# liortalker/MindTheEdge

Measured on AMD Instinct MI355X. Metric: training images/sec, PackNet-SAN+edge-loss 384x1280 bf16, higher is better.
Workload: dtype bf16; 1 GPU; T8: PackNet-SAN + silog + 4-scale depth-edge loss training step, 384x1280, 8 frames/GPU, dropout 0.5, flip 0.5; global_batch=8, height=384, width=1280, parallelism=single GPU

## Files before the change

### include/mte_kernels.h

```cpp
#ifndef MTE_KERNELS_H
#define MTE_KERNELS_H

#ifdef __cplusplus
extern "C" {
#endif

typedef struct ihipStream_t* mte_stream_t;

#define MTE_OK 0
#define MTE_ERR_ARG (-1)
#define MTE_ERR_LAUNCH (-2)
#define MTE_ERR_UNSUPPORTED (-3)
#define MTE_DT_BF16 0
#define MTE_DT_F32 1

#define MTE_CONV_ACCUMULATE 1
#define MTE_CONV_SOLO 2
int mte_conv2d_igemm(const void* x, long ldx, const void* wpack, const float* bias, void* y, long ldy, int out_f32,
                     int B, int H, int W, int Cin_p, int N, int KH, int KW, int dtype,
                     float* workspace, long workspace_elems, int accumulate, mte_stream_t stream);
int mte_conv2d_igemm_unshuffle(const void* x, long ldx, const void* wpack, void* y, long ldy,
                               int B, int H, int W, int Cin_p, int N, int KH, int KW, int dtype, int accumulate, mte_stream_t stream);
#define MTE_OPT_GN_PREZEROED 0
#define MTE_OPT_LOSS_PREZEROED 1
#define MTE_OPT_HANDOFF_FENCES 2
#define MTE_OPT_WGRAD_SHARES_CHIP 3
int mte_set_option(int option, int value);
#define MTE_DEVERR_GN_CLUSTER_FWD 1
#define MTE_DEVERR_GN_CLUSTER_BWD 2
#define MTE_DEVERR_IMAGE_RESAMPLE 4
int mte_device_error_init(void);
int mte_device_error_poll(void);
int mte_conv2d_wgrad(const void* x, long ldx, const void* dy, long ldy, float* dw_stage, int stage_parts, int* parts_out,
                     int B, int H, int W, int Cin_p, int N, int KH, int KW, int dtype, mte_stream_t stream);
int mte_conv2d_wgrad_nine_tap(int H, int W, int Cin_p, int N, int KH, int KW, int dtype);
int mte_pack_conv_weights(const float* w_oihw, void* wfwd, void* wbwd, int Cout, int Cin, int KH, int KW,
                          int Cin_p, int Cout_p, int dtype, mte_stream_t stream);
typedef struct { const float* w; void* wf; void* wb; void* pf; void* pb; int Cout, Cin, taps, Cin_p; int end_f, end_b, end_pf, end_pb; } mte_pack_job;
int mte_pack_conv_weights_multi(const void* jobs, int njobs, int dtype, mte_stream_t stream);
int mte_pack_conv_weights_bwd(const void* wfwd, void* wbwd, int Cout, int KH, int KW, int Cin_p, int dtype, mte_stream_t stream);
int mte_unpack_conv_wgrad(float* dw_stage, int parts, float* dw_oihw, int Cout, int Cin, int KH, int KW, int Cin_p, mte_stream_t stream);
int mte_colsum(const void* y, long ld, long M, int N, float* out, int dtype, mte_stream_t stream);

int mte_conv2d_patch_supported(int W, int Cin_p, int N, int KH, int KW, int dtype);
int mte_conv2d_patch_wgrad_supported(int W, int Cin_p, int N, int KH, int KW, int dtype);
long mte_conv2d_patch_pack_elems(int Cin_p, int N, int KH, int KW);
int mte_conv2d_patch_repack(const void* wgeneric, void* wpatch, int Cin_p, int N, int KH, int KW, mte_stream_t stream);
int mte_conv2d_patch_fwd(const void* x, long ldx, const void* wpatch, const float* bias, void* y, long ldy,
                         int B, int H, int W, int Cin_p, int N, int KH, int KW, int accumulate, mte_stream_t stream);
int mte_conv2d_patch_wgrad(const void* x, long ldx, const void* dy, long lddy, float* dw_stage, int stage_parts, int* parts_out,
                           int B, int H, int W, int Cin_p, int N, int KH, int KW, mte_stream_t stream);
long mte_conv2d_patch_fwd_gn_elems(int B, int H, int W);
int mte_conv2d_patch_fwd_gn(const void* x, long ldx, const void* wpatch, const float* bias, void* y, long ldy, int B, int H, int W, int Cin_p, int N, int KH, int KW,
                            int accumulate, float* rec, long rec_elems, int* tiles_per_sample_out, mte_stream_t stream);

int mte_conv2d_stem_supported(int W, int Cin_p, int N, int KH, int KW, int dtype);
int mte_conv2d_stem_fwd(const void* x, long ldx, const void* wf, const float* bias, void* y, long ldy,
                        int B, int H, int W, int N, int KH, int KW, mte_stream_t stream);
int mte_conv2d_stem_wgrad(const void* x, long ldx, const void* dy, long lddy, float* dw_stage, int stage_parts, int* parts_out,
                          int B, int H, int W, int N, int KH, int KW, mte_stream_t stream);

long mte_gn_stats_elems(int B);
// ... 279 lines not shown
```

### mindtheedge_amd/csrc/conv_igemm.hip

```cpp
#include "common.hpp"
#include "conv_args.hpp"

#ifdef MTE_STAMPS
__device__ unsigned long long g_igemm_stamps[16384 * 8];
extern "C" int mtei_igemm_stamps(unsigned long long* host, int n) {
    return hipMemcpyFromSymbol(host, HIP_SYMBOL(g_igemm_stamps), sizeof(unsigned long long) * n) == hipSuccess ? 0 : -1;
}
#endif

namespace {


template <typename T> struct Mma;
template <> struct Mma<bf16_t> {
    __device__ static __forceinline__ void run(const u32x4_t& a, const u32x4_t& b, f32x16_t& c) {
        c = __builtin_amdgcn_mfma_f32_32x32x16_bf16(__builtin_bit_cast(bf16x8_t, a), __builtin_bit_cast(bf16x8_t, b), c, 0, 0, 0);
    }
};
template <> struct Mma<float> {
    __device__ static __forceinline__ void run(const u32x4_t& a, const u32x4_t& b, f32x16_t& c) {
#pragma unroll
        for (int i = 0; i < 4; ++i)
            c = __builtin_amdgcn_mfma_f32_32x32x2f32(__uint_as_float(a[i]), __uint_as_float(b[i]), c, 0, 0, 0);
    }
// ... 1141 lines not shown

template <typename T>
__global__ __launch_bounds__(256) void pack_weights_bwd_kernel(const T* __restrict__ wf, T* __restrict__ wb,
                                                               int Cout, int taps, int Cin_p, int Cout_p) {
    __shared__ T tile[64][64 + 2];
    const int Kp = taps * Cin_p;
    const int n0 = blockIdx.x * 64, k0 = blockIdx.y * 64;
    for (int i = threadIdx.x; i < 64 * 64; i += 256) {
        const int r = i >> 6, cidx = i & 63;
        const int n = n0 + r, k = k0 + cidx;
        tile[r][cidx] = (n < Cout && k < Kp) ? wf[(long)n * Kp + k] : (T)0;
    }
    __syncthreads();
    for (int i = threadIdx.x; i < 64 * 64; i += 256) {
        const int kk = i >> 6, nn = i & 63;
        const int k = k0 + kk, n = n0 + nn;
        if (k < Kp && n < Cout_p) {
            const int tap = k / Cin_p, c = k - tap * Cin_p;
            wb[((long)c * taps + (taps - 1 - tap)) * Cout_p + n] = n < Cout ? tile[nn][kk] : (T)0;
        }
    }
}

struct PackJob {
    const float* w;
    void* wf;
    void* wb;
    void* pf;
    void* pb;
    int Cout, Cin, taps, Cin_p;
    int end_f, end_b, end_pf, end_pb;
};
constexpr int PACK_JOBS_MAX = 48;
struct PackTable { int n; int pad_; PackJob j[PACK_JOBS_MAX]; };
constexpr int PACK_FRAG_PER_BLOCK = 256 * 8;

template <typename T> __device__ __forceinline__ void store8(T* dst, const float* v);
template <> __device__ __forceinline__ void store8<bf16_t>(bf16_t* dst, const float* v) { *(u32x4_t*)dst = pack16<bf16_t>(v); }
template <> __device__ __forceinline__ void store8<float>(float* dst, const float* v) {
    *(u32x4_t*)dst = pack16<float>(v); *(u32x4_t*)(dst + 4) = pack16<float>(v + 4);
}

__host__ __device__ inline int pack_fn(int taps) { const int f = (64 * 65) / (64 * taps); return f < 1 ? 1 : (f > 16 ? 16 : f); }

template <typename T>
__global__ __launch_bounds__(256) void pack_multi_kernel(const PackTable tb) {
    __shared__ float s_w[64 * 65];
    int ji = 0;
    while (ji + 1 < tb.n && (int)blockIdx.x >= tb.j[ji].end_pb) ++ji;
    const PackJob& J = tb.j[ji];
    const int start = ji ? tb.j[ji - 1].end_pb : 0;
    const int bid = blockIdx.x;
    const int Cout = J.Cout, Cin = J.Cin, taps = J.taps, Cin_p = J.Cin_p;
    const float* __restrict__ w = J.w;
    if (bid < J.end_f) {
        const int fn = pack_fn(taps);
        const int cchunks = (Cin_p + 63) >> 6;
        const int lb = bid - start, n0 = (lb / cchunks) * fn, c0 = (lb - (lb / cchunks) * cchunks) * 64;
        const int nc = min(64, Cin - c0), nn = min(fn, Cout - n0);
        const int run = nc > 0 ? nc * taps : 0, rs = 64 * taps;
        for (int i = threadIdx.x; i < nn * run; i += 256) {
            const int ni = i / run, r = i - ni * run;
            s_w[ni * rs + r] = w[((long)(n0 + ni) * Cin + c0) * taps + r];
        }
        __syncthreads();
        const int ncp = min(64, Cin_p - c0), nch = ncp >> 3;
        T* wf = (T*)J.wf;
        for (int i = threadIdx.x; i < nn * taps * nch; i += 256) {
            const int ch8 = i % nch, t2 = i / nch, tap = t2 % taps, ni = t2 / taps;
            float v[8];
#pragma unroll
            for (int j = 0; j < 8; ++j) {
                const int cl = ch8 * 8 + j;
                v[j] = cl < nc ? s_w[ni * rs + cl * taps + tap] : 0.f;
            }
            store8<T>(wf + ((long)(n0 + ni) * taps + tap) * Cin_p + c0 + ch8 * 8, v);
        }
        return;
    }
    if (bid < J.end_b) {
        const int Kp = taps * Cin_p, Kr = taps * Cin;
        const int ktiles = (Kp + 63) >> 6;
        const int lb = bid - J.end_f, n0 = (lb / ktiles) * 64, k0 = (lb % ktiles) * 64;
        for (int i = threadIdx.x; i < 64 * 64; i += 256) {
            const int r = i >> 6, kk = i & 63;
            const int n = n0 + r, k = k0 + kk;
            s_w[r * 65 + kk] = (n < Cout && k < Kr) ? w[(long)n * Kr + k] : 0.f;
        }
        __syncthreads();
        T* wb = (T*)J.wb;
        if (Cout % 8 == 0) {
            for (int i = threadIdx.x; i < 64 * 8; i += 256) {
                const int kk = i >> 3, n8 = i & 7;
                const int k = k0 + kk, n = n0 + n8 * 8;
                if (k < Kp && n < Cout) {
                    const int c = k / taps, tap = k - c * taps;
                    float v[8];
#pragma unroll
                    for (int j = 0; j < 8; ++j) v[j] = s_w[(n8 * 8 + j) * 65 + kk];
                    store8<T>(wb + ((long)c * taps + (taps - 1 - tap)) * Cout + n, v);
                }
            }
            return;
        }
        for (int i = threadIdx.x; i < 64 * 64; i += 256) {
            const int kk = i >> 6, nn = i & 63;
            const int k = k0 + kk, n = n0 + nn;
            if (k < Kp && n < Cout) {
                const int c = k / taps, tap = k - c * taps;
                Elem<T>::st(wb + ((long)c * taps + (taps - 1 - tap)) * Cout + n, s_w[nn * 65 + kk]);
            }
        }
        return;
    }
    const bool fwd = bid < J.end_pf;
    const int N = fwd ? Cout : Cin_p, C = fwd ? Cin_p : Cout;
    const int NT = (N + 31) >> 5;
    const long total8 = (long)((C + 31) >> 5) * taps * 2 * NT * 64;
    const long i8 = (long)(bid - (fwd ? J.end_b : J.end_pf)) * 256 + threadIdx.x;
    if (i8 >= total8) return;
    long t = i8;
    const int lane = (int)(t & 63); t >>= 6;
    const int nt = (int)(t % NT); t /= NT;
    const int kk = (int)(t & 1); t >>= 1;
    const int tap = (int)(t % taps); const int sl = (int)(t / taps);
    const int n = nt * 32 + (lane & 31), c0 = sl * 32 + kk * 16 + (lane >> 5) * 8;
    float v[8];
#pragma unroll
    for (int j = 0; j < 8; ++j) {
        const int c = c0 + j;
        float x = 0.f;
        if (n < N && c < C) {
            if (fwd) { if (c < Cin) x = w[((long)n * Cin + c) * taps + tap]; }
            else if (n < Cin) x = w[((long)c * Cin + n) * taps + (taps - 1 - tap)];
        }
        v[j] = x;
    }
    store8<T>((T*)(fwd ? J.pf : J.pb) + i8 * 8, v);
}

__global__ __launch_bounds__(256) void unpack_wgrad_kernel(const float* __restrict__ st, float* __restrict__ dw, int Cout, int Cin, int taps, int Cin_p, int parts) {
    extern __shared__ float s_t[];
    const int n = blockIdx.x, c0 = blockIdx.y * 64;
    const int nc = min(64, Cin - c0);
    if (nc <= 0) return;
    const float* src = st + (long)n * taps * Cin_p + c0;
    const long pstride = (long)Cout * taps * Cin_p;
    for (int i = threadIdx.x; i < taps * 16; i += 256) {
        const int tap = i >> 4, c4 = (i & 15) * 4;
        if (c0 + c4 >= Cin_p) continue;
        const float* q = src + (long)tap * Cin_p + c4;
        f32x4_t acc = {0.f, 0.f, 0.f, 0.f};
        int p = 0;
        for (; p + 8 <= parts; p += 8) {
            f32x4_t v[8];
#pragma unroll
            for (int k = 0; k < 8; ++k) v[k] = *(const f32x4_t*)(q + (long)(p + k) * pstride);
#pragma unroll
            for (int k = 0; k < 8; ++k) acc += v[k];
        }
        for (; p < parts; ++p) acc += *(const f32x4_t*)(q + (long)p * pstride);
#pragma unroll
// ... 125 lines not shown
}

int mte_pack_conv_weights(const float* w_oihw, void* wfwd, void* wbwd, int Cout, int Cin, int KH, int KW,
                          int Cin_p, int Cout_p, int dtype, hipStream_t stream) {
    (void)hipGetLastError();
    if (!w_oihw || !wfwd) return MTE_ERR_ARG;
    const int taps = KH * KW;
    if (Cout_p != Cout && wbwd) return MTE_ERR_ARG;
    const dim3 gf(Cout, (Cin_p + 63) / 64), gb((Cout + 63) / 64, (taps * Cin_p + 63) / 64);
    const size_t lds = sizeof(float) * 64 * taps;
    if (dtype == MTE_DT_BF16) {
        hipLaunchKernelGGL(pack_weights_fwd_kernel<bf16_t>, gf, dim3(256), lds, stream, w_oihw, (bf16_t*)wfwd, Cout, Cin, taps, Cin_p);
        if (wbwd) hipLaunchKernelGGL(pack_weights_bwd_kernel<bf16_t>, gb, dim3(256), 0, stream, (const bf16_t*)wfwd, (bf16_t*)wbwd, Cout, taps, Cin_p, Cout_p);
    } else {
        hipLaunchKernelGGL(pack_weights_fwd_kernel<float>, gf, dim3(256), lds, stream, w_oihw, (float*)wfwd, Cout, Cin, taps, Cin_p);
        if (wbwd) hipLaunchKernelGGL(pack_weights_bwd_kernel<float>, gb, dim3(256), 0, stream, (const float*)wfwd, (float*)wbwd, Cout, taps, Cin_p, Cout_p);
    }
    return mte_check_launch();
}

int mte_pack_conv_weights_multi(const void* jobs_host, int njobs, int dtype, hipStream_t stream) {
    (void)hipGetLastError();
    if (!jobs_host || njobs < 0 || (dtype != MTE_DT_BF16 && dtype != MTE_DT_F32)) return MTE_ERR_ARG;
    const PackJob* src = (const PackJob*)jobs_host;
    for (int j0 = 0; j0 < njobs; j0 += PACK_JOBS_MAX) {
        PackTable tb{};
        tb.n = njobs - j0 < PACK_JOBS_MAX ? njobs - j0 : PACK_JOBS_MAX;
        long blocks = 0;
        for (int i = 0; i < tb.n; ++i) {
            PackJob J = src[j0 + i];
            if (!J.w || !J.wf || J.taps < 1 || J.taps > 49 || J.Cin_p % 8 != 0 || J.Cin > J.Cin_p) return MTE_ERR_ARG;
            if ((J.pf || J.pb) && dtype != MTE_DT_BF16) return MTE_ERR_ARG;
            if (J.pb && !J.wb) return MTE_ERR_ARG;
            blocks += (long)((J.Cout + pack_fn(J.taps) - 1) / pack_fn(J.taps)) * ((J.Cin_p + 63) / 64);
            J.end_f = (int)blocks;
            if (J.wb) blocks += (long)((J.Cout + 63) / 64) * ((J.taps * J.Cin_p + 63) / 64);
            J.end_b = (int)blocks;
            if (J.pf) blocks += ((long)((J.Cin_p + 31) / 32) * J.taps * 2 * ((J.Cout + 31) / 32) * 64 + 255) / 256;
            J.end_pf = (int)blocks;
            if (J.pb) blocks += ((long)((J.Cout + 31) / 32) * J.taps * 2 * ((J.Cin_p + 31) / 32) * 64 + 255) / 256;
            J.end_pb = (int)blocks;
            if (blocks > 0x7fffffffL) return MTE_ERR_UNSUPPORTED;
            tb.j[i] = J;
        }
        if (blocks == 0) continue;
        if (dtype == MTE_DT_BF16) hipLaunchKernelGGL(pack_multi_kernel<bf16_t>, dim3((unsigned)blocks), dim3(256), 0, stream, tb);
        else hipLaunchKernelGGL(pack_multi_kernel<float>, dim3((unsigned)blocks), dim3(256), 0, stream, tb);
    }
    return mte_check_launch();
}

int mte_pack_conv_weights_bwd(const void* wfwd, void* wbwd, int Cout, int KH, int KW, int Cin_p, int dtype, hipStream_t stream) {
    (void)hipGetLastError();
    if (!wfwd || !wbwd) return MTE_ERR_ARG;
    const int taps = KH * KW;
    const dim3 gb((Cout + 63) / 64, (taps * Cin_p + 63) / 64);
    if (dtype == MTE_DT_BF16) hipLaunchKernelGGL(pack_weights_bwd_kernel<bf16_t>, gb, dim3(256), 0, stream, (const bf16_t*)wfwd, (bf16_t*)wbwd, Cout, taps, Cin_p, Cout);
    else hipLaunchKernelGGL(pack_weights_bwd_kernel<float>, gb, dim3(256), 0, stream, (const float*)wfwd, (float*)wbwd, Cout, taps, Cin_p, Cout);
    return mte_check_launch();
}

int mte_unpack_conv_wgrad(float* dw_stage, int parts, float* dw_oihw, int Cout, int Cin, int KH, int KW, int Cin_p, hipStream_t stream) {
    (void)hipGetLastError();
    if (!dw_stage || !dw_oihw || parts < 1) return MTE_ERR_ARG;
    const dim3 grid(Cout, (Cin + 63) / 64);
    if (parts > 32) {
        const long elems = (long)Cout * KH * KW * Cin_p;
        const int pc = ((parts + 31) / 32 + RP_PC - 1) / RP_PC * RP_PC;
        const int groups = (parts + pc - 1) / pc;
        hipLaunchKernelGGL(reduce_parts_kernel, dim3((unsigned)((elems / 4 + 255) / 256), (unsigned)groups), dim3(256), 0, stream, dw_stage, elems, parts, pc);
        dw_stage += (long)parts * elems;
        parts = groups;
// ... 22 lines not shown
```

### mindtheedge_amd/kernels.py

```python
import ctypes
import itertools
import math
import os
import weakref

import torch

from ._lib import lib, MteError

DT_BF16, DT_F32 = 0, 1
_state = {"compute_dtype": torch.bfloat16, "weights_epoch": 0}


def set_compute_dtype(dtype):
    dtype = {"bf16": torch.bfloat16, "fp32": torch.float32, "f32": torch.float32}.get(dtype, dtype)
    assert dtype in (torch.bfloat16, torch.float32)
    _state["compute_dtype"] = dtype


def compute_dtype():
    return _state["compute_dtype"]


def bump_weights_epoch():
# ... 301 lines not shown
            self.pkey = self.key
        if which == 'f':
            if not self.pf_ok:
                self._patch_pack(w, 'f')
                self.pf_ok = True
            return self.pf
        if not self.pb_ok:
            self._patch_pack(w, 'b')
            self.pb_ok = True
        return self.pb

    pf_ok = pb_ok = False
    _want_pf = _want_pb = False

    def _pack(self, w, dtype, need_bwd):
        cout, cin, kh, kw = w.shape
        cin_p = round8(cin)
        dtc = DT_BF16 if dtype == torch.bfloat16 else DT_F32
        if self.wf is None or self.wf.dtype != dtype or tuple(self.wf.shape) != (cout, kh * kw, cin_p):
            self.wf = torch.empty((cout, kh * kw, cin_p), dtype=dtype, device=w.device)
            self.wb = None
        if need_bwd and (self.wb is None or self.wb.dtype != dtype):
            self.wb = torch.empty((cin_p, kh * kw, cout), dtype=dtype, device=w.device)
        lib.mte_pack_conv_weights(w.detach().contiguous().data_ptr(), self.wf.data_ptr(), _ptr(self.wb) if need_bwd else 0,
                                  cout, cin, kh, kw, cin_p, cout, dtc, _stream())
        self.has_bwd = bool(need_bwd)

    has_bwd = False

    def get(self, w, dtype, need_bwd):
        key = (w.data_ptr(), w._version, weights_epoch(), dtype, tuple(w.shape))
        self._last = (weakref.ref(w), dtype)
        self._order = next(WeightPack._seq)
        if key != self.key:
            if self._event is not None:
                torch.cuda.current_stream().wait_event(self._event)
            self._event = None
            self._pack(w, dtype, need_bwd)
            self.key = key
        else:
            self._sync_prefetch()
            if need_bwd and not self.has_bwd:
                cout, cin, kh, kw = w.shape
                cin_p = round8(cin)
                if self.wb is None:
                    self.wb = torch.empty((cin_p, kh * kw, cout), dtype=dtype, device=w.device)
                lib.mte_pack_conv_weights_bwd(self.wf.data_ptr(), self.wb.data_ptr(), cout, kh, kw, cin_p,
                                              DT_BF16 if dtype == torch.bfloat16 else DT_F32, _stream())
                self.has_bwd = True
        return self.wf, (self.wb if self.has_bwd else None)


class _PackJob(ctypes.Structure):
    _fields_ = [("w", ctypes.c_void_p), ("wf", ctypes.c_void_p), ("wb", ctypes.c_void_p), ("pf", ctypes.c_void_p), ("pb", ctypes.c_void_p),
                ("Cout", ctypes.c_int), ("Cin", ctypes.c_int), ("taps", ctypes.c_int), ("Cin_p", ctypes.c_int),
                ("end_f", ctypes.c_int), ("end_b", ctypes.c_int), ("end_pf", ctypes.c_int), ("end_pb", ctypes.c_int)]


_PACK_CHUNKS = (16, 48)
_pack_jobs = {"sig": None, "chunks": []}


def _pack_job_chunks(packs):
    sig = (len(packs),) + tuple((id(pk), pk._last[0]().data_ptr(), pk.wf.data_ptr(), _ptr(pk.wb) if pk.has_bwd else 0,
                                 _ptr(pk.pf) if pk._want_pf else 0, _ptr(pk.pb) if pk._want_pb else 0) for pk in packs)
    if _pack_jobs["sig"] == sig:
        return _pack_jobs["chunks"]
    chunks = []
    for dt in (torch.bfloat16, torch.float32):
        part = [pk for pk in packs if pk._last[1] == dt and pk.wf is not None and pk.wf.dtype == dt]
        i = 0
        while i < len(part):
            group = part[i:i + (_PACK_CHUNKS[0] if i == 0 else _PACK_CHUNKS[1])]
            i += len(group)
            arr = (_PackJob * len(group))()
            for o, pk in zip(arr, group):
                w = pk._last[0]()
                cout, cin, kh, kw = w.shape
                o.w, o.wf = w.data_ptr(), pk.wf.data_ptr()
                o.wb = pk.wb.data_ptr() if pk.has_bwd else None
                o.pf = pk.pf.data_ptr() if pk._want_pf else None
                o.pb = pk.pb.data_ptr() if pk._want_pb else None
                o.Cout, o.Cin, o.taps, o.Cin_p = cout, cin, kh * kw, round8(cin)
            chunks.append((arr, len(group), DT_BF16 if dt == torch.bfloat16 else DT_F32, group))
    _pack_jobs["sig"], _pack_jobs["chunks"] = sig, chunks
    return chunks


def prefetch_weight_packs():
    packs = []
    for r in WeightPack._live:
        pk = r()
        if pk is not None and pk._last is not None and pk.key is not None and pk._last[0]() is not None and pk._last[0]().is_cuda:
            packs.append(pk)
    WeightPack._live = [r for r in WeightPack._live if r() is not None]
    if not packs:
        return
    packs.sort(key=lambda pk: pk._order)
    if _side["enabled"]:
        if not _side["streams"]:
            _side["streams"] = [_new_side_stream() for _ in range(max(1, _SIDE_STREAMS))]
        side = _side["streams"][0]
        ev = torch.cuda.Event()
        ev.record()
        side.wait_event(ev)
    else:
        side = torch.cuda.current_stream()
    with torch.cuda.stream(side):
        _refold_all()
        _refresh_main_weights(packs)
        for pk in packs:
            pk._want_pf = pk.pf_ok and pk.pkey == pk.key and pk.pf is not None
            pk._want_pb = pk.pb_ok and pk.pkey == pk.key and pk.pb is not None and pk.has_bwd
        st = _stream()
        odd = [pk for pk in packs if not (pk._last[0]().is_contiguous() and pk._last[0]().dtype == torch.float32)]
        if odd:
            packs = [pk for pk in packs if pk not in odd]
            for pk in odd:
                w, dtype = pk._last[0](), pk._last[1]
                pk._pack(w, dtype, pk.has_bwd)
                pk.key = (w.data_ptr(), w._version, weights_epoch(), dtype, tuple(w.shape))
                pk.pkey, pk.pf_ok, pk.pb_ok, pk._event = None, False, False, None
        for arr, n, dtc, group in _pack_job_chunks(packs):
            lib.mte_pack_conv_weights_multi(ctypes.addressof(arr), n, dtc, st)
            ev = None
            if _side["enabled"]:
                ev = torch.cuda.Event()
                ev.record(side)
            for pk in group:
                w, dtype = pk._last[0](), pk._last[1]
                pk.key = (w.data_ptr(), w._version, weights_epoch(), dtype, tuple(w.shape))
                pk.pkey = pk.key
                pk.pf_ok, pk.pb_ok = pk._want_pf, pk._want_pb
                pk._event = ev
    if _side["enabled"] and torch.cuda.is_current_stream_capturing():
        torch.cuda.current_stream().wait_stream(side)
        for pk in packs:
            pk._event = None


SPLITK_SLABS = 8
_splitk_ws = {}


def _splitk_workspace(M, N, device):
    tiles = ((M + 127) // 128) * ((N + 127) // 128)
    if tiles >= 384:
        return None, 0
    n = SPLITK_SLABS * M * N
    if torch.cuda.is_current_stream_capturing():
        return torch.empty((n,), dtype=torch.float32, device=device), n
    key = (str(device), _stream())
    ws = _splitk_ws.get(key)
    if ws is None or ws.numel() < n:
        ws = _splitk_ws[key] = torch.empty((n,), dtype=torch.float32, device=device)
    return ws, n

# ... 155 lines not shown
    dyp, lddy = _pl(dy)
    xp, ldx = _pl(x)
    st = _stream()
    dbias = None
    per = cout * kh * kw * Cp
    patch = _cfg["patch_kernels"] and x.dtype == torch.bfloat16 and lib.mte_conv2d_patch_wgrad_supported(W, Cp, cout, kh, kw, DT_BF16) == 1
    if patch and lib.mte_conv2d_wgrad_nine_tap(H, W, Cp, cout, kh, kw, _dt(x)) == 1:
        patch = False
    if kh * kw == 1 and Cp >= 64:
        patch = False
    wide = 256 if per <= (1 << 18) else (64 if per <= (1 << 19) else 32)
    cap = max(1, min(512, (192 << 20) // (4 * per))) if patch and _cfg["patch_wgrad_slabs"] else max(1, min(wide, (96 << 20) // (4 * per)))
    stem = _stem_ok(W, Cp, cout, kh, kw, x.dtype)
    if stem:
        cap = 2048
    stage = torch.empty((cap + (32 if cap > 32 else 0), cout, kh * kw, Cp), dtype=torch.float32, device=x.device)
    parts = ctypes.c_int(1)
    if stem:
        lib.mte_conv2d_stem_wgrad(xp, ldx, dyp, lddy, stage.data_ptr(), cap, ctypes.byref(parts), B, H, W, cout, kh, kw, st)
    elif patch:
        lib.mte_conv2d_patch_wgrad(xp, ldx, dyp, lddy, stage.data_ptr(), cap, ctypes.byref(parts), B, H, W, Cp, cout, kh, kw, st)
    else:
        lib.mte_conv2d_wgrad(xp, ldx, dyp, lddy, stage.data_ptr(), cap, ctypes.byref(parts), B, H, W, Cp, cout, kh, kw, _dt(x), st)
    dw = dw_out if dw_out is not None else torch.empty_like(w, dtype=torch.float32)
    lib.mte_unpack_conv_wgrad(stage.data_ptr(), parts.value, dw.data_ptr(), cout, cin, kh, kw, Cp, st)
    if need_dbias:
        dbias = dbias_out if dbias_out is not None else torch.empty((cout,), dtype=torch.float32, device=x.device)
        lib.mte_colsum(dyp, lddy, B * H * W, cout, dbias.data_ptr(), _dt(dy), st)
    return dw, dbias


def conv_backward(x, dy, w, pack, need_dx, need_dw=True, need_dbias=True, dw_out=None, dbias_out=None, fork_slot=None, sunk=False, sites=None):
    dw = dbias = dx = None
    on_side = False
    if need_dw:
        sunk = bool(sunk) and dw_out is not None and (dbias_out is not None or not need_dbias)
        on_side = sunk and _side["enabled"] and need_dx

    def wgrad():
        if on_side:
            if _side["keep_bytes"] > _SIDE_KEEP_LIMIT:
                join_side_stream()
            with torch.cuda.stream(_side_stream_for(x, dy)):
                return _conv_wgrad(x, dy, w, need_dbias, dw_out, dbias_out)
        return _conv_wgrad(x, dy, w, need_dbias, dw_out, dbias_out)

    if need_dw:
# ... 130 lines not shown
        recs = []
        y = conv_forward(x, wf, b, cout, kh, kw, pack=pack, w=w, gn_records=recs)
        z, stats = _gn_forward(y, None, None, gamma, beta, GN_EPS, out=None if out is None else alias_of(out), records=recs)
        ctx.save_for_backward(x, w, y, stats, gamma, beta)
        ctx.pack = pack
        ctx.bias = b
        return z

    @staticmethod
    def backward(ctx, dz):
        x, w, y, stats, gamma, beta = ctx.saved_tensors
        b = ctx.bias
        gg, sg = _grad_dst(gamma, zero=True)
        gb, sb = _grad_dst(beta, zero=True)
        gbias, sbias = _grad_dst(b, zero=True)
        gw, sw = _grad_dst(w)
        dy, _, dgamma, dbeta, db = _gn_backward(dz, y, None, None, stats, gamma, beta, GN_EPS, False, want_dbias=True,
                                                dgamma=gg, dbeta=gb, dbias=gbias)
        dx, dw, _ = conv_backward(x, dy, w, ctx.pack, ctx.needs_input_grad[0], need_dbias=False, dw_out=gw, fork_slot=ctx.fork_slot, sunk=sw)
        return dx, _grad_ret(w, dw, sw), _grad_ret(b, db, sbias), _grad_ret(gamma, dgamma, sg), _grad_ret(beta, dbeta, sb), None, None


def _main_weight(pack, w, cm):
    key = (w.data_ptr(), w._version, weights_epoch())
    wm = getattr(pack, "_main_w", None)
    if wm is None or tuple(wm.shape) != (w.shape[0], cm, w.shape[2], w.shape[3]) or wm.device != w.device:
        wm = pack._main_w = torch.empty((w.shape[0], cm, w.shape[2], w.shape[3]), dtype=torch.float32, device=w.device)
        pack._main_key = None
    pack._main_src = (weakref.ref(w), cm)
    if pack._main_key != key:
        wm.copy_(w.detach()[:, :cm])
        pack._main_key = key
    return wm


def _refresh_main_weights(packs):
    for pk in packs:
        src = getattr(pk, "_main_src", None)
        wm = getattr(pk, "_main_w", None)
        if src is None or wm is None:
            continue
        w = src[0]()
        if w is None or tuple(wm.shape) != (w.shape[0], src[1], w.shape[2], w.shape[3]):
            continue
        key = (w.data_ptr(), w._version, weights_epoch())
        if pk._main_key != key:
            wm.copy_(w.detach()[:, :src[1]])
            pk._main_key = key


class ConvGnEluInvFn(torch.autograd.Function):

    @staticmethod
    def forward(ctx, x, inv, w, b, gamma, beta, pack, out=None):
        ctx.fork_slot = getattr(x, "_mte_fork_slot", None)
        cout, cin, kh, kw = w.shape
        cm = cin - 1
        B, Cp, H, W = x.shape
        if (kh, kw) != (3, 3) or Cp != cm or tuple(inv.shape) != (B, 1, H // 2, W // 2):
            raise MteError("rank-1 inverse-depth term: expected a 3x3 layer over %d + 1 channels and a [B,1,H/2,W/2] map, got %s / %s / %s"
                           % (Cp, tuple(w.shape), tuple(x.shape), tuple(inv.shape)))
        wm = _main_weight(pack, w, cm)
        wf, _ = pack.get(wm, x.dtype, bool(ctx.needs_input_grad[0]))
        invc = inv.detach().contiguous().float()
        y = new_act(B, cout, H, W, x.dtype, x.device)
        yp, ldy = _pl(y)
        w1 = w.detach().data_ptr() + 4 * cm * 9
        xp, ldx = _pl(x)
        if (_cfg["fuse_inv_term"] and pack is not None and _patch_ok(W, Cp, cout, kh, kw, x.dtype)
                and lib.mte_conv2d_patch_fwd_rank1_ok(_ptr(b), ldx, B, H, W, Cp, cout) == 1):
            lib.mte_conv2d_patch_fwd_rank1(xp, ldx, pack.get_patch(wm, 'f').data_ptr(), _ptr(b), yp, ldy, B, H, W, Cp, cout,
# ... 332 lines not shown
    f["params"] = tuple(weakref.ref(t) for t in (w, w3, b, b3))
    if f["key"] != _fold_key(w, w3, b, b3) or _FOLD_INLINE:
        _fold_now(f, w, w3, b, b3)
        pack_fold.key = f["pk_r"].key = f["pk_c"].key = None
    return f["Wf"], f["bf"]


_FOLD_INLINE = bool(os.environ.get("MTE_FOLD_INLINE"))
_fold_hooks = []


def _refold_all():
    live = []
    for r in _fold_hooks:
        pk = r()
        f = getattr(pk, "fold", None) if pk is not None else None
        if f is None:
            continue
        live.append(r)
        ps = [p() for p in f.get("params", ())]
        if len(ps) == 4 and all(p is not None for p in ps) and f["key"] != _fold_key(*ps):
            _fold_now(f, *ps)
    _fold_hooks[:] = live


_unshuffle_ok = {}


def _dgrad_unshuffled(dy, Wf, pack, dx, k):
    B, C, H, W = dx.shape
    cp = dy.shape[1]
    if dy.dtype != torch.bfloat16 or 4 * C > 256 or os.environ.get("MTE_NO_UNSHUFFLE") == "1":
        return False
    key = (B, H // 2, W // 2, cp, 4 * C, k)
    ok = _unshuffle_ok.get(key)
    if ok is False:
        return False
    _, wb = pack.get(Wf, dy.dtype, True)
    dyp, lddy = _pl(dy)
    dxp, lddx = _pl(dx)
    args = (dyp, lddy, wb.data_ptr(), dxp, lddx, B, H // 2, W // 2, cp, 4 * C, k, k, _dt(dy), 0, _stream())
    if ok is None:
        from . import _lib as _L
        rc = _L.lib.load().mte_conv2d_igemm_unshuffle(*args)
        if rc not in (0, -3):
            raise MteError("mte_conv2d_igemm_unshuffle failed: %s" % rc)
# ... 357 lines not shown
```

Baseline: 376.9 images/sec.

## Unify weight-pack kernel into single LDS-tiled pass and pack strided master slices directly

```diff
diff --git a/include/mte_kernels.h b/include/mte_kernels.h
--- a/include/mte_kernels.h
+++ b/include/mte_kernels.h
@@ -38,6 +38,8 @@
                           int Cin_p, int Cout_p, int dtype, mte_stream_t stream);
 typedef struct { const float* w; void* wf; void* wb; void* pf; void* pb; int Cout, Cin, taps, Cin_p; int end_f, end_b, end_pf, end_pb; } mte_pack_job;
 int mte_pack_conv_weights_multi(const void* jobs, int njobs, int dtype, mte_stream_t stream);
+typedef struct { const float* w; void* wf; void* wb; void* pf; void* pb; int Cout, Cin, taps, Cin_p; int Cin_total; int end; } mte_pack_job_v2;
+int mte_pack_conv_weights_multi_v2(const void* jobs, int njobs, int dtype, mte_stream_t stream);
 int mte_pack_conv_weights_bwd(const void* wfwd, void* wbwd, int Cout, int KH, int KW, int Cin_p, int dtype, mte_stream_t stream);
 int mte_unpack_conv_wgrad(float* dw_stage, int parts, float* dw_oihw, int Cout, int Cin, int KH, int KW, int Cin_p, mte_stream_t stream);
 int mte_colsum(const void* y, long ld, long M, int N, float* out, int dtype, mte_stream_t stream);
diff --git a/mindtheedge_amd/csrc/conv_igemm.hip b/mindtheedge_amd/csrc/conv_igemm.hip
--- a/mindtheedge_amd/csrc/conv_igemm.hip
+++ b/mindtheedge_amd/csrc/conv_igemm.hip
@@ -1187,122 +1187,7 @@
     }
 }
 
-struct PackJob {
-    const float* w;
-    void* wf;
-    void* wb;
-    void* pf;
-    void* pb;
-    int Cout, Cin, taps, Cin_p;
-    int end_f, end_b, end_pf, end_pb;
-};
-constexpr int PACK_JOBS_MAX = 48;
-struct PackTable { int n; int pad_; PackJob j[PACK_JOBS_MAX]; };
-constexpr int PACK_FRAG_PER_BLOCK = 256 * 8;
-
-template <typename T> __device__ __forceinline__ void store8(T* dst, const float* v);
-template <> __device__ __forceinline__ void store8<bf16_t>(bf16_t* dst, const float* v) { *(u32x4_t*)dst = pack16<bf16_t>(v); }
-template <> __device__ __forceinline__ void store8<float>(float* dst, const float* v) {
-    *(u32x4_t*)dst = pack16<float>(v); *(u32x4_t*)(dst + 4) = pack16<float>(v + 4);
-}
-
-__host__ __device__ inline int pack_fn(int taps) { const int f = (64 * 65) / (64 * taps); return f < 1 ? 1 : (f > 16 ? 16 : f); }
-
-template <typename T>
-__global__ __launch_bounds__(256) void pack_multi_kernel(const PackTable tb) {
-    __shared__ float s_w[64 * 65];
-    int ji = 0;
-    while (ji + 1 < tb.n && (int)blockIdx.x >= tb.j[ji].end_pb) ++ji;
-    const PackJob& J = tb.j[ji];
-    const int start = ji ? tb.j[ji - 1].end_pb : 0;
-    const int bid = blockIdx.x;
-    const int Cout = J.Cout, Cin = J.Cin, taps = J.taps, Cin_p = J.Cin_p;
-    const float* __restrict__ w = J.w;
-    if (bid < J.end_f) {
-        const int fn = pack_fn(taps);
-        const int cchunks = (Cin_p + 63) >> 6;
-        const int lb = bid - start, n0 = (lb / cchunks) * fn, c0 = (lb - (lb / cchunks) * cchunks) * 64;
-        const int nc = min(64, Cin - c0), nn = min(fn, Cout - n0);
-        const int run = nc > 0 ? nc * taps : 0, rs = 64 * taps;
-        for (int i = threadIdx.x; i < nn * run; i += 256) {
-            const int ni = i / run, r = i - ni * run;
-            s_w[ni * rs + r] = w[((long)(n0 + ni) * Cin + c0) * taps + r];
-        }
-        __syncthreads();
-        const int ncp = min(64, Cin_p - c0), nch = ncp >> 3;
-        T* wf = (T*)J.wf;
-        for (int i = threadIdx.x; i < nn * taps * nch; i += 256) {
-            const int ch8 = i % nch, t2 = i / nch, tap = t2 % taps, ni = t2 / taps;
-            float v[8];
-#pragma unroll
-            for (int j = 0; j < 8; ++j) {
-                const int cl = ch8 * 8 + j;
-                v[j] = cl < nc ? s_w[ni * rs + cl * taps + tap] : 0.f;
-            }
-            store8<T>(wf + ((long)(n0 + ni) * taps + tap) * Cin_p + c0 + ch8 * 8, v);
-        }
-        return;
-    }
-    if (bid < J.end_b) {
-        const int Kp = taps * Cin_p, Kr = taps * Cin;
-        const int ktiles = (Kp + 63) >> 6;
-        const int lb = bid - J.end_f, n0 = (lb / ktiles) * 64, k0 = (lb % ktiles) * 64;
-        for (int i = threadIdx.x; i < 64 * 64; i += 256) {
-            const int r = i >> 6, kk = i & 63;
-            const int n = n0 + r, k = k0 + kk;
-            s_w[r * 65 + kk] = (n < Cout && k < Kr) ? w[(long)n * Kr + k] : 0.f;
-        }
-        __syncthreads();
-        T* wb = (T*)J.wb;
-        if (Cout % 8 == 0) {
-            for (int i = threadIdx.x; i < 64 * 8; i += 256) {
-                const int kk = i >> 3, n8 = i & 7;
-                const int k = k0 + kk, n = n0 + n8 * 8;
-                if (k < Kp && n < Cout) {
-                    const int c = k / taps, tap = k - c * taps;
-                    float v[8];
-#pragma unroll
-                    for (int j = 0; j < 8; ++j) v[j] = s_w[(n8 * 8 + j) * 65 + kk];
-                    store8<T>(wb + ((long)c * taps + (taps - 1 - tap)) * Cout + n, v);
-                }
-            }
-            return;
-        }
-        for (int i = threadIdx.x; i < 64 * 64; i += 256) {
-            const int kk = i >> 6, nn = i & 63;
-            const int k = k0 + kk, n = n0 + nn;
-            if (k < Kp && n < Cout) {
-                const int c = k / taps, tap = k - c * taps;
-                Elem<T>::st(wb + ((long)c * taps + (taps - 1 - tap)) * Cout + n, s_w[nn * 65 + kk]);
-            }
-        }
-        return;
-    }
-    const bool fwd = bid < J.end_pf;
-    const int N = fwd ? Cout : Cin_p, C = fwd ? Cin_p : Cout;
-    const int NT = (N + 31) >> 5;
-    const long total8 = (long)((C + 31) >> 5) * taps * 2 * NT * 64;
-    const long i8 = (long)(bid - (fwd ? J.end_b : J.end_pf)) * 256 + threadIdx.x;
-    if (i8 >= total8) return;
-    long t = i8;
-    const int lane = (int)(t & 63); t >>= 6;
-    const int nt = (int)(t % NT); t /= NT;
-    const int kk = (int)(t & 1); t >>= 1;
-    const int tap = (int)(t % taps); const int sl = (int)(t / taps);
-    const int n = nt * 32 + (lane & 31), c0 = sl * 32 + kk * 16 + (lane >> 5) * 8;
-    float v[8];
-#pragma unroll
-    for (int j = 0; j < 8; ++j) {
-        const int c = c0 + j;
-        float x = 0.f;
-        if (n < N && c < C) {
-            if (fwd) { if (c < Cin) x = w[((long)n * Cin + c) * taps + tap]; }
-            else if (n < Cin) x = w[((long)c * Cin + n) * taps + (taps - 1 - tap)];
-        }
-        v[j] = x;
-    }
-    store8<T>((T*)(fwd ? J.pf : J.pb) + i8 * 8, v);
-}
+#include "pack_multi.hpp"
 
 __global__ __launch_bounds__(256) void unpack_wgrad_kernel(const float* __restrict__ st, float* __restrict__ dw, int Cout, int Cin, int taps, int Cin_p, int parts) {
     extern __shared__ float s_t[];
@@ -1474,32 +1359,24 @@
 int mte_pack_conv_weights_multi(const void* jobs_host, int njobs, int dtype, hipStream_t stream) {
     (void)hipGetLastError();
     if (!jobs_host || njobs < 0 || (dtype != MTE_DT_BF16 && dtype != MTE_DT_F32)) return MTE_ERR_ARG;
-    const PackJob* src = (const PackJob*)jobs_host;
+    const PackJobV1* src = (const PackJobV1*)jobs_host;
     for (int j0 = 0; j0 < njobs; j0 += PACK_JOBS_MAX) {
-        PackTable tb{};
-        tb.n = njobs - j0 < PACK_JOBS_MAX ? njobs - j0 : PACK_JOBS_MAX;
-        long blocks = 0;
-        for (int i = 0; i < tb.n; ++i) {
-            PackJob J = src[j0 + i];
-            if (!J.w || !J.wf || J.taps < 1 || J.taps > 49 || J.Cin_p % 8 != 0 || J.Cin > J.Cin_p) return MTE_ERR_ARG;
-            if ((J.pf || J.pb) && dtype != MTE_DT_BF16) return MTE_ERR_ARG;
-            if (J.pb && !J.wb) return MTE_ERR_ARG;
-            blocks += (long)((J.Cout + pack_fn(J.taps) - 1) / pack_fn(J.taps)) * ((J.Cin_p + 63) / 64);
-            J.end_f = (int)blocks;
-            if (J.wb) blocks += (long)((J.Cout + 63) / 64) * ((J.taps * J.Cin_p + 63) / 64);
-            J.end_b = (int)blocks;
-            if (J.pf) blocks += ((long)((J.Cin_p + 31) / 32) * J.taps * 2 * ((J.Cout + 31) / 32) * 64 + 255) / 256;
-            J.end_pf = (int)blocks;
-            if (J.pb) blocks += ((long)((J.Cout + 31) / 32) * J.taps * 2 * ((J.Cin_p + 31) / 32) * 64 + 255) / 256;
-            J.end_pb = (int)blocks;
-            if (blocks > 0x7fffffffL) return MTE_ERR_UNSUPPORTED;
-            tb.j[i] = J;
-        }
-        if (blocks == 0) continue;
-        if (dtype == MTE_DT_BF16) hipLaunchKernelGGL(pack_multi_kernel<bf16_t>, dim3((unsigned)blocks), dim3(256), 0, stream, tb);
-        else hipLaunchKernelGGL(pack_multi_kernel<float>, dim3((unsigned)blocks), dim3(256), 0, stream, tb);
-    }
-    return mte_check_launch();
+        PackJob jobs[PACK_JOBS_MAX];
+        const int n = njobs - j0 < PACK_JOBS_MAX ? njobs - j0 : PACK_JOBS_MAX;
+        for (int i = 0; i < n; ++i) {
+            const PackJobV1& s = src[j0 + i];
+            jobs[i] = PackJob{s.w, s.wf, s.wb, s.pf, s.pb, s.Cout, s.Cin, s.taps, s.Cin_p, s.Cin, 0};
+        }
+        const int rc = pack_multi_launch(jobs, n, dtype, stream);
+        if (rc != MTE_OK) return rc;
+    }
+    return MTE_OK;
+}
+
+int mte_pack_conv_weights_multi_v2(const void* jobs_host, int njobs, int dtype, hipStream_t stream) {
+    (void)hipGetLastError();
+    if (!jobs_host || njobs < 0 || (dtype != MTE_DT_BF16 && dtype != MTE_DT_F32)) return MTE_ERR_ARG;
+    return pack_multi_launch((const PackJob*)jobs_host, njobs, dtype, stream);
 }
 
 int mte_pack_conv_weights_bwd(const void* wfwd, void* wbwd, int Cout, int KH, int KW, int Cin_p, int dtype, hipStream_t stream) {
diff --git a/mindtheedge_amd/csrc/pack_multi.hpp b/mindtheedge_amd/csrc/pack_multi.hpp
--- /dev/null
+++ b/mindtheedge_amd/csrc/pack_multi.hpp
@@ -0,0 +1,166 @@
+#pragma once
+
+struct PackJob {
+    const float* w;
+    void* wf;
+    void* wb;
+    void* pf;
+    void* pb;
+    int Cout, Cin, taps, Cin_p;
+    int Cin_total;
+    int end;
+};
+struct PackJobV1 {
+    const float* w; void* wf; void* wb; void* pf; void* pb;
+    int Cout, Cin, taps, Cin_p;
+    int end_f, end_b, end_pf, end_pb;
+};
+constexpr int PACK_JOBS_MAX = 48;
+struct PackTable { int n; int pad_; PackJob j[PACK_JOBS_MAX]; };
+static_assert(sizeof(PackTable) <= 4096, "the job table travels as a kernel argument");
+
+constexpr int PACK_LDS_BYTES = 52 * 1024;
+constexpr int PACK_ROW_PAD = 2;
+
+struct PackTile { int nt, cc; };
+__host__ __device__ inline PackTile pack_tile(int taps, int elem_size) {
+    int nt = 64, cc = 64;
+    while (nt * (cc * taps + PACK_ROW_PAD) * elem_size > PACK_LDS_BYTES && cc > 8) {
+        if (nt >= cc && nt > 8) nt >>= 1;
+        else cc >>= 1;
+    }
+    return {nt, cc};
+}
+__host__ __device__ inline int pack_next(const PackJob& J) { return (J.pf || J.pb) ? (J.Cout + 31) & ~31 : J.Cout; }
+__host__ __device__ inline int pack_cext(const PackJob& J) { return (J.pf || J.pb) ? (J.Cin_p + 31) & ~31 : J.Cin_p; }
+__host__ __device__ inline long pack_blocks(const PackJob& J, int elem_size) {
+    const PackTile t = pack_tile(J.taps, elem_size);
+    return (long)((pack_next(J) + t.nt - 1) / t.nt) * ((pack_cext(J) + t.cc - 1) / t.cc);
+}
+
+template <typename T> __device__ __forceinline__ void store8t(T* dst, const T* v);
+template <> __device__ __forceinline__ void store8t<bf16_t>(bf16_t* dst, const bf16_t* v) {
+    u32x4_t c;
+#pragma unroll
+    for (int i = 0; i < 4; ++i) c[i] = (unsigned)v[2 * i] | ((unsigned)v[2 * i + 1] << 16);
+    *(u32x4_t*)dst = c;
+}
+template <> __device__ __forceinline__ void store8t<float>(float* dst, const float* v) {
+    u32x4_t a, b;
+#pragma unroll
+    for (int i = 0; i < 4; ++i) { a[i] = __float_as_uint(v[i]); b[i] = __float_as_uint(v[4 + i]); }
+    *(u32x4_t*)dst = a; *(u32x4_t*)(dst + 4) = b;
+}
+
+template <typename T>
+__global__ __launch_bounds__(256) void pack_multi_kernel(const PackTable tb) {
+    __shared__ T s_w[PACK_LDS_BYTES / sizeof(T)];
+    int ji = 0;
+    while (ji + 1 < tb.n && (int)blockIdx.x >= tb.j[ji].end) ++ji;
+    const PackJob& J = tb.j[ji];
+    const int lb = (int)blockIdx.x - (ji ? tb.j[ji - 1].end : 0);
+    const int Cout = J.Cout, Cin = J.Cin, taps = J.taps, Cin_p = J.Cin_p;
+    const PackTile tl = pack_tile(taps, (int)sizeof(T));
+    const int NT = tl.nt, CC = tl.cc, RS = CC * taps + PACK_ROW_PAD;
+    const int ctiles = (pack_cext(J) + CC - 1) / CC;
+    const int n0 = (lb / ctiles) * NT, c0 = (lb % ctiles) * CC;
+    const int nn = max(0, min(NT, Cout - n0));
+    const int nc = max(0, min(CC, Cin - c0));
+    const int ncp = max(0, min(CC, Cin_p - c0));
+
+    {
+        const int wave = threadIdx.x >> 6, lane = threadIdx.x & 63;
+        const int run = nc * taps, row_len = CC * taps;
+        for (int ni = wave; ni < NT; ni += 4) {
+            T* row = s_w + ni * RS;
+            const int live = ni < nn ? run : 0;
+            const float* __restrict__ src = J.w + ((long)(n0 + ni) * J.Cin_total + c0) * taps;
+#pragma unroll 4
+            for (int r = lane; r < live; r += 64) Elem<T>::st(row + r, src[r]);
+            for (int r = live + lane; r < row_len; r += 64) row[r] = (T)0;
+        }
+    }
+    __syncthreads();
+
+    const int nch = ncp >> 3;
+    if (nn > 0 && nch > 0) {
+        T* wf = (T*)J.wf;
+        for (int i = threadIdx.x; i < nn * taps * nch; i += 256) {
+            const int ch8 = i % nch, t2 = i / nch, tap = t2 % taps, ni = t2 / taps;
+            T v[8];
+#pragma unroll
+            for (int j = 0; j < 8; ++j) v[j] = s_w[ni * RS + (ch8 * 8 + j) * taps + tap];
+            store8t<T>(wf + ((long)(n0 + ni) * taps + tap) * Cin_p + c0 + ch8 * 8, v);
+        }
+    }
+    if (J.wb && nn > 0 && ncp > 0) {
+        T* wb = (T*)J.wb;
+        const int nk = ncp * taps;
+        if (Cout % 8 == 0) {
+            const int n8c = nn >> 3;
+            for (int i = threadIdx.x; i < nk * n8c; i += 256) {
+                const int n8 = i % n8c, k = i / n8c, cl = k / taps, tap = k - cl * taps;
+                T v[8];
+#pragma unroll
+                for (int j = 0; j < 8; ++j) v[j] = s_w[(n8 * 8 + j) * RS + k];
+                store8t<T>(wb + ((long)(c0 + cl) * taps + (taps - 1 - tap)) * Cout + n0 + n8 * 8, v);
+            }
+        } else {
+            for (int i = threadIdx.x; i < nk * nn; i += 256) {
+                const int nl = i % nn, k = i / nn, cl = k / taps, tap = k - cl * taps;
+                wb[((long)(c0 + cl) * taps + (taps - 1 - tap)) * Cout + n0 + nl] = s_w[nl * RS + k];
+            }
+        }
+    }
+    if (J.pf) {
+        T* pf = (T*)J.pf;
+        const int NTf = (Cout + 31) >> 5, slices = (Cin_p + 31) >> 5, c8s = CC >> 3;
+        for (int i = threadIdx.x; i < NT * c8s * taps; i += 256) {
+            const int nl = i % NT, t2 = i / NT, ch8 = t2 % c8s, tap = t2 / c8s;
+            const int n = n0 + nl, c = c0 + ch8 * 8;
+            if (n >= NTf * 32 || c >= slices * 32) continue;
+            T v[8];
+#pragma unroll
+            for (int j = 0; j < 8; ++j) v[j] = s_w[nl * RS + (ch8 * 8 + j) * taps + tap];
+            const long i8 = ((((long)(c >> 5) * taps + tap) * 2 + ((c >> 4) & 1)) * NTf + (n >> 5)) * 64 + ((c >> 3) & 1) * 32 + (n & 31);
+            store8t<T>(pf + i8 * 8, v);
+        }
+    }
+    if (J.pb) {
+        T* pb = (T*)J.pb;
+        const int NTb = (Cin_p + 31) >> 5, slices = (Cout + 31) >> 5, n8s = NT >> 3;
+        for (int i = threadIdx.x; i < CC * n8s * taps; i += 256) {
+            const int cl = i % CC, t2 = i / CC, n8 = t2 % n8s, tap = t2 / n8s;
+            const int c = c0 + cl, n = n0 + n8 * 8;
+            if (c >= NTb * 32 || n >= slices * 32) continue;
+            T v[8];
+#pragma unroll
+            for (int j = 0; j < 8; ++j) v[j] = s_w[(n8 * 8 + j) * RS + cl * taps + (taps - 1 - tap)];
+            const long i8 = ((((long)(n >> 5) * taps + tap) * 2 + ((n >> 4) & 1)) * NTb + (c >> 5)) * 64 + ((n >> 3) & 1) * 32 + (c & 31);
+            store8t<T>(pb + i8 * 8, v);
+        }
+    }
+}
+
+inline int pack_multi_launch(const PackJob* jobs, int njobs, int dtype, hipStream_t stream) {
+    const int es = dtype == MTE_DT_BF16 ? 2 : 4;
+    for (int j0 = 0; j0 < njobs; j0 += PACK_JOBS_MAX) {
+        PackTable tb{};
+        tb.n = njobs - j0 < PACK_JOBS_MAX ? njobs - j0 : PACK_JOBS_MAX;
+        long blocks = 0;
+        for (int i = 0; i < tb.n; ++i) {
+            PackJob J = jobs[j0 + i];
+            if (!J.w || !J.wf || J.Cout < 0 || J.Cin < 0 || J.taps < 1 || J.taps > 49 || J.Cin_p % 8 != 0 || J.Cin > J.Cin_p || J.Cin_total < J.Cin) return MTE_ERR_ARG;
+            if ((J.pf || J.pb) && dtype != MTE_DT_BF16) return MTE_ERR_ARG;
+            if (J.pb && !J.wb) return MTE_ERR_ARG;
+            blocks += pack_blocks(J, es);
+            if (blocks > 0x7fffffffL) return MTE_ERR_UNSUPPORTED;
+            J.end = (int)blocks;
+            tb.j[i] = J;
+        }
+        if (blocks == 0) continue;
+        if (dtype == MTE_DT_BF16) hipLaunchKernelGGL(pack_multi_kernel<bf16_t>, dim3((unsigned)blocks), dim3(256), 0, stream, tb);
+        else hipLaunchKernelGGL(pack_multi_kernel<float>, dim3((unsigned)blocks), dim3(256), 0, stream, tb);
+    }
+    return mte_check_launch();
+}
diff --git a/mindtheedge_amd/kernels.py b/mindtheedge_amd/kernels.py
--- a/mindtheedge_amd/kernels.py
+++ b/mindtheedge_amd/kernels.py
@@ -347,8 +347,14 @@
             self.wb = None
         if need_bwd and (self.wb is None or self.wb.dtype != dtype):
             self.wb = torch.empty((cin_p, kh * kw, cout), dtype=dtype, device=w.device)
-        lib.mte_pack_conv_weights(w.detach().contiguous().data_ptr(), self.wf.data_ptr(), _ptr(self.wb) if need_bwd else 0,
-                                  cout, cin, kh, kw, cin_p, cout, dtc, _stream())
+        ct = _master_stride(w)
+        if ct is not None and ct != cin:
+            job = (_PackJob * 1)()
+            _fill_pack_job(job[0], w, ct, self.wf, self.wb if need_bwd else None, None, None)
+            lib.mte_pack_conv_weights_multi_v2(ctypes.addressof(job), 1, dtc, _stream())
+        else:
+            lib.mte_pack_conv_weights(w.detach().contiguous().data_ptr(), self.wf.data_ptr(), _ptr(self.wb) if need_bwd else 0,
+                                      cout, cin, kh, kw, cin_p, cout, dtc, _stream())
         self.has_bwd = bool(need_bwd)
 
     has_bwd = False
@@ -379,35 +385,57 @@
 class _PackJob(ctypes.Structure):
     _fields_ = [("w", ctypes.c_void_p), ("wf", ctypes.c_void_p), ("wb", ctypes.c_void_p), ("pf", ctypes.c_void_p), ("pb", ctypes.c_void_p),
                 ("Cout", ctypes.c_int), ("Cin", ctypes.c_int), ("taps", ctypes.c_int), ("Cin_p", ctypes.c_int),
-                ("end_f", ctypes.c_int), ("end_b", ctypes.c_int), ("end_pf", ctypes.c_int), ("end_pb", ctypes.c_int)]
+                ("Cin_total", ctypes.c_int), ("end", ctypes.c_int)]
+
+
+def _master_stride(w):
+    if w.dtype != torch.float32 or w.dim() != 4:
+        return None
+    cout, cin, kh, kw = w.shape
+    if w.is_contiguous():
+        return cin
+    taps = kh * kw
+    s0, s1, s2, s3 = w.stride()
+    if (s1, s2, s3) == (taps, kw, 1) and s0 % taps == 0 and s0 // taps >= cin:
+        return s0 // taps
+    return None
+
+
+def _fill_pack_job(o, w, cin_total, wf, wb, pf, pb):
+    cout, cin, kh, kw = w.shape
+    o.w, o.wf = w.data_ptr(), wf.data_ptr()
+    o.wb = wb.data_ptr() if wb is not None else None
+    o.pf = pf.data_ptr() if pf is not None else None
+    o.pb = pb.data_ptr() if pb is not None else None
+    o.Cout, o.Cin, o.taps, o.Cin_p, o.Cin_total = cout, cin, kh * kw, round8(cin), cin_total
 
 
 _PACK_CHUNKS = (16, 48)
+_PACK_FOLDS_FIRST = os.environ.get("MTE_PACK_FOLDS_FIRST") == "1"
 _pack_jobs = {"sig": None, "chunks": []}
 
 
-def _pack_job_chunks(packs):
-    sig = (len(packs),) + tuple((id(pk), pk._last[0]().data_ptr(), pk.wf.data_ptr(), _ptr(pk.wb) if pk.has_bwd else 0,
-                                 _ptr(pk.pf) if pk._want_pf else 0, _ptr(pk.pb) if pk._want_pb else 0) for pk in packs)
+def _pack_job_chunks(packs, folded):
+    sig = (len(packs), _PACK_FOLDS_FIRST) + tuple((id(pk), pk._last[0]().data_ptr(), pk.wf.data_ptr(), _ptr(pk.wb) if pk.has_bwd else 0,
+                                                   _ptr(pk.pf) if pk._want_pf else 0, _ptr(pk.pb) if pk._want_pb else 0,
+                                                   pk._last[0]().data_ptr() in folded) for pk in packs)
     if _pack_jobs["sig"] == sig:
         return _pack_jobs["chunks"]
     chunks = []
-    for dt in (torch.bfloat16, torch.float32):
-        part = [pk for pk in packs if pk._last[1] == dt and pk.wf is not None and pk.wf.dtype == dt]
-        i = 0
-        while i < len(part):
-            group = part[i:i + (_PACK_CHUNKS[0] if i == 0 else _PACK_CHUNKS[1])]
-            i += len(group)
-            arr = (_PackJob * len(group))()
-            for o, pk in zip(arr, group):
-                w = pk._last[0]()
-                cout, cin, kh, kw = w.shape
-                o.w, o.wf = w.data_ptr(), pk.wf.data_ptr()
-                o.wb = pk.wb.data_ptr() if pk.has_bwd else None
-                o.pf = pk.pf.data_ptr() if pk._want_pf else None
-                o.pb = pk.pb.data_ptr() if pk._want_pb else None
-                o.Cout, o.Cin, o.taps, o.Cin_p = cout, cin, kh * kw, round8(cin)
-            chunks.append((arr, len(group), DT_BF16 if dt == torch.bfloat16 else DT_F32, group))
+    for late in ((None,) if _PACK_FOLDS_FIRST else (False, True)):
+        for dt in (torch.bfloat16, torch.float32):
+            part = [pk for pk in packs if pk._last[1] == dt and pk.wf is not None and pk.wf.dtype == dt
+                    and (late is None or (pk._last[0]().data_ptr() in folded) == late)]
+            i = 0
+            while i < len(part):
+                group = part[i:i + (_PACK_CHUNKS[0] if i == 0 and not late else _PACK_CHUNKS[1])]
+                i += len(group)
+                arr = (_PackJob * len(group))()
+                for o, pk in zip(arr, group):
+                    w = pk._last[0]()
+                    _fill_pack_job(o, w, _master_stride(w), pk.wf, pk.wb if pk.has_bwd else None,
+                                   pk.pf if pk._want_pf else None, pk.pb if pk._want_pb else None)
+                chunks.append((arr, len(group), DT_BF16 if dt == torch.bfloat16 else DT_F32, group, bool(late)))
     _pack_jobs["sig"], _pack_jobs["chunks"] = sig, chunks
     return chunks
 
@@ -432,22 +460,30 @@
     else:
         side = torch.cuda.current_stream()
     with torch.cuda.stream(side):
-        _refold_all()
-        _refresh_main_weights(packs)
         for pk in packs:
             pk._want_pf = pk.pf_ok and pk.pkey == pk.key and pk.pf is not None
             pk._want_pb = pk.pb_ok and pk.pkey == pk.key and pk.pb is not None and pk.has_bwd
         st = _stream()
-        odd = [pk for pk in packs if not (pk._last[0]().is_contiguous() and pk._last[0]().dtype == torch.float32)]
-        if odd:
-            packs = [pk for pk in packs if pk not in odd]
+        odd = [pk for pk in packs if _master_stride(pk._last[0]()) is None]
+        packs = [pk for pk in packs if pk not in odd]
+        folds_done = False
+
+        def folds_and_odd():
+            _refold_all()
             for pk in odd:
                 w, dtype = pk._last[0](), pk._last[1]
                 pk._pack(w, dtype, pk.has_bwd)
                 pk.key = (w.data_ptr(), w._version, weights_epoch(), dtype, tuple(w.shape))
                 pk.pkey, pk.pf_ok, pk.pb_ok, pk._event = None, False, False, None
-        for arr, n, dtc, group in _pack_job_chunks(packs):
-            lib.mte_pack_conv_weights_multi(ctypes.addressof(arr), n, dtc, st)
+
+        if _PACK_FOLDS_FIRST:
+            folds_and_odd()
+            folds_done = True
+        for arr, n, dtc, group, after_folds in _pack_job_chunks(packs, _fold_masters()):
+            if after_folds and not folds_done:
+                folds_and_odd()
+                folds_done = True
+            lib.mte_pack_conv_weights_multi_v2(ctypes.addressof(arr), n, dtc, st)
             ev = None
             if _side["enabled"]:
                 ev = torch.cuda.Event()
@@ -458,6 +494,8 @@
                 pk.pkey = pk.key
                 pk.pf_ok, pk.pb_ok = pk._want_pf, pk._want_pb
                 pk._event = ev
+        if not folds_done:
+            folds_and_odd()
     if _side["enabled"] and torch.cuda.is_current_stream_capturing():
         torch.cuda.current_stream().wait_stream(side)
         for pk in packs:
@@ -659,7 +697,7 @@
         lib.mte_conv2d_patch_wgrad(xp, ldx, dyp, lddy, stage.data_ptr(), cap, ctypes.byref(parts), B, H, W, Cp, cout, kh, kw, st)
     else:
         lib.mte_conv2d_wgrad(xp, ldx, dyp, lddy, stage.data_ptr(), cap, ctypes.byref(parts), B, H, W, Cp, cout, kh, kw, _dt(x), st)
-    dw = dw_out if dw_out is not None else torch.empty_like(w, dtype=torch.float32)
+    dw = dw_out if dw_out is not None else torch.empty(tuple(w.shape), dtype=torch.float32, device=w.device)
     lib.mte_unpack_conv_wgrad(stage.data_ptr(), parts.value, dw.data_ptr(), cout, cin, kh, kw, Cp, st)
     if need_dbias:
         dbias = dbias_out if dbias_out is not None else torch.empty((cout,), dtype=torch.float32, device=x.device)
@@ -836,31 +874,8 @@
 
 
 def _main_weight(pack, w, cm):
-    key = (w.data_ptr(), w._version, weights_epoch())
-    wm = getattr(pack, "_main_w", None)
-    if wm is None or tuple(wm.shape) != (w.shape[0], cm, w.shape[2], w.shape[3]) or wm.device != w.device:
-        wm = pack._main_w = torch.empty((w.shape[0], cm, w.shape[2], w.shape[3]), dtype=torch.float32, device=w.device)
-        pack._main_key = None
-    pack._main_src = (weakref.ref(w), cm)
-    if pack._main_key != key:
-        wm.copy_(w.detach()[:, :cm])
-        pack._main_key = key
+    wm = pack._main_w = w.detach()[:, :cm]
     return wm
-
-
-def _refresh_main_weights(packs):
-    for pk in packs:
-        src = getattr(pk, "_main_src", None)
-        wm = getattr(pk, "_main_w", None)
-        if src is None or wm is None:
-            continue
-        w = src[0]()
-        if w is None or tuple(wm.shape) != (w.shape[0], src[1], w.shape[2], w.shape[3]):
-            continue
-        key = (w.data_ptr(), w._version, weights_epoch())
-        if pk._main_key != key:
-            wm.copy_(w.detach()[:, :src[1]])
-            pk._main_key = key
 
 
 class ConvGnEluInvFn(torch.autograd.Function):
@@ -1239,6 +1254,15 @@
         if len(ps) == 4 and all(p is not None for p in ps) and f["key"] != _fold_key(*ps):
             _fold_now(f, *ps)
     _fold_hooks[:] = live
+
+
+def _fold_masters():
+    ptrs = set()
+    for r in _fold_hooks:
+        f = getattr(r(), "fold", None)
+        if f is not None:
+            ptrs.update(f[k].data_ptr() for k in ("Wf", "Wr", "Wc"))
+    return ptrs
 
 
 _unshuffle_ok = {}
```

Result: no change. 379.4 images/sec, median of 6 (+0.6%).
